# ChuWeiEr/GravInv3DHMC

Measured on AMD Instinct MI355X. Metric: HMC leapfrog steps/sec + G·ρ achieved HBM GB/s at 1/2/4/8 GPUs, higher is better.
Workload: dtype f64

## Files before the change

### gravinv3dhmc_amd/csrc/fold.hip.h

```cpp
#pragma once

namespace ghk {

struct FoldArgs {
    const double *S;
    const int *obs_img;
    const int *cell_orbit;
    int nF, ldF;
    int64_t n_orb;
    int64_t orb_per_team;
    int n_pp;
    int64_t N;
};

typedef const d2 __attribute__((address_space(1))) *gconst_d2ptr;

__global__ void __launch_bounds__(256) fold_build_kernel(const double *G, int64_t ld, FoldArgs f, double *S,
                                                         unsigned long long *dev_bits)
{
    __shared__ double red[2][4];
    const int64_t o = blockIdx.x;
    const int n = 4 * f.ldF;
    int co[4];
#pragma unroll
    for (int g = 0; g < 4; ++g) co[g] = f.cell_orbit[4 * o + g];
    double dev = 0.0, amax = 0.0;
    for (int e = threadIdx.x; e < n; e += blockDim.x) {
        const int i = e >> 2, k = e & 3;
        double mean = 0.0;
        if (i < f.nF) {
            double v[4];
#pragma unroll
            for (int g = 0; g < 4; ++g) v[g] = G[(int64_t)co[k ^ g] * ld + f.obs_img[4 * i + g]];
            mean = (((v[0] + v[1]) + v[2]) + v[3]) * 0.25;
#pragma unroll
            for (int g = 0; g < 4; ++g) dev = fmax(dev, fabs(v[g] - mean));
            amax = fmax(amax, fabs(mean));
        }
        S[o * n + e] = mean;
    }
#pragma unroll
    for (int off = 32; off >= 1; off >>= 1) {
        dev = fmax(dev, __shfl_xor(dev, off, WAVE));
        amax = fmax(amax, __shfl_xor(amax, off, WAVE));
    }
    const int lane = threadIdx.x & 63, wave = threadIdx.x >> 6;
    if (lane == 0) {
        red[0][wave] = dev;
        red[1][wave] = amax;
    }
    __syncthreads();
    if (threadIdx.x == 0) {
        for (int w = 1; w < (int)(blockDim.x >> 6); ++w) {
            dev = fmax(dev, red[0][w]);
            amax = fmax(amax, red[1][w]);
        }
        const double rel = amax > 0.0 ? dev / amax : 0.0;
        atomicMax(dev_bits, (unsigned long long)__double_as_longlong(rel));
    }
}

__device__ __forceinline__ double readlane_d(double v, int l)
{
    const long long b = __double_as_longlong(v);
    const int lo = __builtin_amdgcn_readlane((int)b, l);
    const int hi = __builtin_amdgcn_readlane((int)(b >> 32), l);
    return __longlong_as_double(((long long)hi << 32) | (long long)(unsigned)lo);
}

template <int EPT2>
struct FoldCol {
    d2 v[EPT2];
    int j;
    int jn;
    double cv;
};

constexpr int FOLD_SLOT = 16 * 16 + 8;

enum { FOLD_IN_X = 0, FOLD_IN_P, FOLD_IN_GREG, FOLD_IN_HI, FOLD_IN_LO, FOLD_IN_PN, FOLD_IN_GACC, FOLD_IN_N };

template <int CTRL>
__device__ __forceinline__ double dpp_mov(double v)
{
    const long long b = __double_as_longlong(v);
    const int lo = __builtin_amdgcn_update_dpp(0, (int)b, CTRL, 0xf, 0xf, false);
    const int hi = __builtin_amdgcn_update_dpp(0, (int)(b >> 32), CTRL, 0xf, 0xf, false);
    return __longlong_as_double(((long long)hi << 32) | (long long)(unsigned)lo);
}

template <int Q>
__device__ __forceinline__ double dpp_from_up(double v)
{
    const long long b = __double_as_longlong(v);
    const int lo = __builtin_amdgcn_update_dpp(0, (int)b, 0x100 | Q, 0xf, 0xf, false);
    const int hi = __builtin_amdgcn_update_dpp(0, (int)(b >> 32), 0x100 | Q, 0xf, 0xf, false);
    return __longlong_as_double(((long long)hi << 32) | (long long)(unsigned)lo);
}

template <int EPT2>
__global__ void __launch_bounds__(1024) fold_sweep_kernel(SweepArgs a, FoldArgs f)
{
    constexpr int TT = 1024, NW = 16;
    extern __shared__ __attribute__((aligned(16))) double smem[];
    double *rF = smem;
    double *scratch = smem + 4 * f.ldF;

    const int tid = threadIdx.x;
    const int lane = tid & 63;
    const int wave = tid >> 6;
    const int n2 = 2 * f.ldF;
    const int mode = a.mode;

    if (mode & SW_ADJ) {
        for (int e = tid; e < 4 * f.ldF; e += TT) rF[e] = (e >> 2) < f.nF ? a.r[f.obs_img[e]] : 0.0;
    }
    __syncthreads();

    const int64_t ob = (int64_t)blockIdx.x * f.orb_per_team;
    int64_t oend = ob + f.orb_per_team;
    if (oend > f.n_orb) oend = f.n_orb;
    const int cnt = ob < oend ? (int)(oend - ob) : 0;

    d2 acc[EPT2][2];
#pragma unroll
    for (int k = 0; k < EPT2; ++k) acc[k][0] = acc[k][1] = d2{0.0, 0.0};
    double pp = 0.0;

    unsigned voff = (unsigned)tid * (unsigned)sizeof(d2);
    unsigned coff_last;
    {
        const int e = (EPT2 - 1) * TT + tid;
        coff_last = (unsigned)(e < n2 ? e : n2 - 1) * (unsigned)sizeof(d2);
    }
    const bool last_in = (EPT2 - 1) * TT + tid < n2;
    const int hl = (lane >> 3) & 3, ql = lane & 7;
    const double *in_base = ql == FOLD_IN_P      ? a.p_in
                            : ql == FOLD_IN_GREG ? a.greg
                            : ql == FOLD_IN_HI   ? a.high
                            : ql == FOLD_IN_LO   ? a.low
                            : ql == FOLD_IN_PN   ? a.pn_in
                            : (ql == FOLD_IN_GACC && (mode & SW_GACC)) ? a.g_out
                                                                       : a.x_in;
    const int lastc = cnt - 1;
    auto orb = [&](int i) -> int64_t { return ob + (i < lastc ? i : lastc); };
    auto load_col = [&](FoldCol<EPT2> &c, int64_t o, int64_t o_after) {
        const int jn = f.cell_orbit[4 * o_after + hl];
        const unsigned long long col = (unsigned long long)(f.S + o * (int64_t)(4 * f.ldF));
#pragma unroll
        for (int k = 0; k < EPT2 - 1; ++k) {
            unsigned long long colk = col + (unsigned long long)k * TT * sizeof(d2);
            asm volatile("" : "+s"(colk));
            asm volatile("" : "+v"(voff));
            c.v[k] = __builtin_nontemporal_load(reinterpret_cast<gconst_d2ptr>(colk + voff));
        }
        asm volatile("" : "+v"(coff_last));
        c.v[EPT2 - 1] = __builtin_nontemporal_load(reinterpret_cast<gconst_d2ptr>(col + coff_last));
        asm volatile("" : "+v"(c.jn)::"memory");
        c.j = c.jn;
        c.cv = in_base[c.j];
        c.jn = jn;
    };

    auto process = [&](const FoldCol<EPT2> &cur, int it) {
        double xl = cur.cv;
        const double pl = dpp_from_up<FOLD_IN_P>(cur.cv);
        double xh[4];
        if (mode & SW_ADJ) {
            const d2 *rF2 = reinterpret_cast<const d2 *>(rF) + 2 * (tid >> 1);
            double u0 = 0.0, u1 = 0.0, u2 = 0.0, u3 = 0.0;
#pragma unroll
            for (int k = 0; k < EPT2; ++k) {
                if (k < EPT2 - 1 || last_in) {
                    const d2 ra = rF2[k * TT], rb = rF2[k * TT + 1];
                    const d2 v = cur.v[k];
                    u0 += v.x * ra.x;
                    u0 += v.y * ra.y;
                    u1 += v.x * ra.y;
                    u1 += v.y * ra.x;
                    u2 += v.x * rb.x;
                    u2 += v.y * rb.y;
                    u3 += v.x * rb.y;
                    u3 += v.y * rb.x;
                }
            }
            const bool odd = (tid & 1) != 0, hi2 = (tid & 2) != 0;
            const double w0 = odd ? u2 : u0, w1 = odd ? u3 : u1, w2 = odd ? u0 : u2, w3 = odd ? u1 : u3;
            const double a0 = (odd ? w2 : w0) + dpp_mov<0xb1>(odd ? w0 : w2);
            const double a1 = (odd ? w3 : w1) + dpp_mov<0xb1>(odd ? w1 : w3);
            double sq = (hi2 ? a1 : a0) + dpp_mov<0x4e>(hi2 ? a0 : a1);
            sq = dpp_add<0x114, 0xf>(sq);
            sq = dpp_add<0x118, 0xf>(sq);
            double *slot = scratch + (it & 1) * FOLD_SLOT;
            if ((lane & 15) >= 12) slot[wave * 16 + (((lane & 1) << 1) | ((lane >> 1) & 1)) * 4 + (lane >> 4)] = sq;
            __syncthreads();
            const d2 *sl = reinterpret_cast<const d2 *>(slot + (lane >> 2) * 16 + (lane & 3) * 4);
            const d2 ra = sl[0], rb = sl[1];
            double sv = (ra.x + ra.y) + (rb.x + rb.y);
            sv = dpp_add<0x114, 0xf>(sv);
            sv = dpp_add<0x118, 0xf>(sv);
            double t[4];
#pragma unroll
            for (int h = 0; h < 4; ++h)
                t[h] = ((readlane_d(sv, 12 + h) + readlane_d(sv, 28 + h)) + readlane_d(sv, 44 + h)) + readlane_d(sv, 60 + h);
            const double th = hl == 0 ? t[0] : hl == 1 ? t[1] : hl == 2 ? t[2] : t[3];
            const double g = 2.0 * th + dpp_from_up<FOLD_IN_GREG>(cur.cv);
            double pv = 0.0, pf = 0.0;
            if (mode & SW_PFIN) {
                pf = pl - a.c_p * g;
                pv = pf;
            }
            if (mode & SW_UPD) {
                const double chi = dpp_from_up<FOLD_IN_HI>(cur.cv), clo = dpp_from_up<FOLD_IN_LO>(cur.cv);
                const double psrc = (mode & SW_SPEC) ? dpp_from_up<FOLD_IN_PN>(cur.cv) : pl;
                double pj = psrc - a.c_u * g;
                double xj = xl + a.dt * pj;
                if (xj > chi) {
                    xj = chi;
                    pj = -pj;
                } else if (xj < clo) {
                    xj = clo;
                    pj = -pj;
                }
                pv = pj;
                xl = xj;
            }
            if (mode & SW_PFIN) {
#pragma unroll
                for (int h = 0; h < 4; ++h) {
                    const double q = readlane_d(pf, 8 * h);
                    pp += q * q;
                }
            }
            if (tid < 32 && ql == 0) {
                const int j = cur.j;
                if (mode & SW_GOUT) a.g_out[j] = (mode & SW_GACC) ? dpp_from_up<FOLD_IN_GACC>(cur.cv) + g : g;
                if (mode & SW_UPD) {
                    a.p_out[j] = pv;
                    a.x_out[j] = xl;
                } else if ((mode & SW_PFIN) && !(mode & SW_SPEC)) {
                    a.p_out[j] = pv;
                }
            }
        }
        if (mode & SW_FWD) {
#pragma unroll
            for (int h = 0; h < 4; ++h) xh[h] = readlane_d(xl, 8 * h);
#pragma unroll
            for (int k = 0; k < EPT2; ++k) {
                const d2 v = cur.v[k];
                acc[k][0].x += v.x * xh[0];
                acc[k][0].x += v.y * xh[1];
                acc[k][0].y += v.x * xh[1];
                acc[k][0].y += v.y * xh[0];
                acc[k][1].x += v.x * xh[2];
                acc[k][1].x += v.y * xh[3];
                acc[k][1].y += v.x * xh[3];
                acc[k][1].y += v.y * xh[2];
            }
        }
#pragma unroll
        for (int k = 0; k < EPT2; ++k) asm volatile("" ::"v"(cur.v[k]));
    };

    if (cnt > 0) {
        FoldCol<EPT2> b0, b1;
        b0.jn = f.cell_orbit[4 * orb(0) + hl];
        b1.jn = f.cell_orbit[4 * orb(1) + hl];
        load_col(b0, orb(0), orb(2));
        int i = 0;
        for (;;) {
            load_col(b1, orb(i + 1), orb(i + 3));
            process(b0, i);
            if (++i >= cnt) break;
            load_col(b0, orb(i + 1), orb(i + 3));
            process(b1, i);
            if (++i >= cnt) break;
        }
    }

    if ((mode & SW_PFIN) && tid == 0) {
        a.pp_part[blockIdx.x] = pp;
        for (int t = (int)(blockIdx.x + gridDim.x); t < f.n_pp; t += (int)gridDim.x) a.pp_part[t] = 0.0;
    }

    if (mode & SW_FWD) {
        double *out = a.slab + (int64_t)blockIdx.x * a.ld;
        double ds = 0.0;
#pragma unroll
        for (int k = 0; k < EPT2; ++k) {
            const int e = k * TT + tid;
            const double p2 = __shfl_xor(acc[k][1].x, 1, WAVE), p3 = __shfl_xor(acc[k][1].y, 1, WAVE);
            const double tA = acc[k][0].x + p2, tB = acc[k][0].y + p3;
            const int i = e >> 1;
            if (e < n2 && i < f.nF) {
                const int m2 = 2 * (tid & 1);
                out[f.obs_img[4 * i + m2]] = tA;
                out[f.obs_img[4 * i + m2 + 1]] = tB;
                ds += tA;
                ds += tB;
            }
        }
        for (int64_t e = f.N + tid; e < a.ld; e += TT) out[e] = 0.0;
        if (a.dsum) {
            const double t = block_allreduce_sum(ds, scratch, NW);
            if (tid == 0) a.dsum[blockIdx.x] = t;
        }
    }
}


struct FoldPairArgs {
    const int *wtab;
    const int *ptab;
    int64_t n_work, work_per_team;
};
constexpr int FOLD_PAIR_W = 16;
constexpr int FOLD_PSLOT = 64;

constexpr int fold_pair_slots(int rows) { return (rows - 1) / 2; }
constexpr int fold_pair_cols(int rows) { return 2 * (rows - fold_pair_slots(rows)); }

__global__ void __launch_bounds__(512) fold_pair_rows_kernel(FoldArgs f, const int *code, double *S)
{
    extern __shared__ __attribute__((aligned(16))) double smem[];
    const int n = 4 * f.ldF;
    double *blk = S + (int64_t)blockIdx.x * n;
    for (int e = threadIdx.x; e < n; e += blockDim.x) smem[e] = blk[e];
    __syncthreads();
    for (int e = threadIdx.x; e < n; e += blockDim.x) {
        const int cd = code[e >> 2];
        const int k = e >> 11, t = (e >> 2) & 511, w = min(512, f.ldF - 512 * k);
        blk[2048 * k + 2 * (((e >> 1) & 1) * w + t) + (e & 1)] = cd >= 0 ? smem[(cd & ~3) | ((e ^ cd) & 3)] : 0.0;
    }
}

__global__ void __launch_bounds__(256) fold_pair_mean_kernel(FoldArgs f, const int *row_tau, const int *orb_tau, double *S,
                                                             unsigned long long *dev_bits)
{
    __shared__ double red[2][4];
    const int64_t o = blockIdx.x;
    const int ot = orb_tau[o];
    const int64_t o2 = ot >> 2;
    const int co = ot & 3;
    const int n = 4 * f.nF;
    const int64_t ldb = 4 * (int64_t)f.ldF;
    double dev = 0.0, amax = 0.0;
    if (o <= o2) {
        for (int e = threadIdx.x; e < n; e += blockDim.x) {
            const int k = e & 3, rt = row_tau[e >> 2];
            const int ks = ((k & 1) << 1) | (k >> 1);
            const int e2 = (rt & ~3) | (ks ^ co ^ (rt & 3));
            if (o < o2 || e < e2) {
                const double u = S[o * ldb + e], v = S[o2 * ldb + e2];
                const double m = (u + v) * 0.5;
                S[o * ldb + e] = m;
                S[o2 * ldb + e2] = m;
                dev = fmax(dev, fabs(u - m));
                amax = fmax(amax, fabs(m));
            } else if (e == e2) {
                amax = fmax(amax, fabs(S[o * ldb + e]));
            }
        }
    }
#pragma unroll
    for (int off = 32; off >= 1; off >>= 1) {
        dev = fmax(dev, __shfl_xor(dev, off, WAVE));
        amax = fmax(amax, __shfl_xor(amax, off, WAVE));
    }
    const int lane = threadIdx.x & 63, wave = threadIdx.x >> 6;
    if (lane == 0) {
        red[0][wave] = dev;
        red[1][wave] = amax;
    }
    __syncthreads();
    if (threadIdx.x == 0) {
        for (int w = 1; w < (int)(blockDim.x >> 6); ++w) {
            dev = fmax(dev, red[0][w]);
            amax = fmax(amax, red[1][w]);
        }
        const double rel = amax > 0.0 ? dev / amax : 0.0;
        atomicMax(dev_bits, (unsigned long long)__double_as_longlong(rel));
    }
}

template <int ROWS>
struct FoldPairCol {
    d2 v[ROWS][2];
    int j;
    int jn, on;
    bool live;
    double cv;
};

template <int ROWS>
__global__ void __launch_bounds__(512) fold_pair_sweep_kernel(SweepArgs a, FoldArgs f, FoldPairArgs p)
{
    constexpr int TT = 512, NW = 8;
    constexpr int NP = fold_pair_slots(ROWS), NS = ROWS - NP, NC = fold_pair_cols(ROWS);
    extern __shared__ __attribute__((aligned(16))) double smem[];
    double *rL = smem;
    double *scratch = smem + NC * TT * 4;

    const int tid = threadIdx.x;
    const int lane = tid & 63;
    const int wave = tid >> 6;
    const int mode = a.mode;

    if (mode & SW_ADJ) {
        for (int e = tid; e < NC * TT * 4; e += TT) {
            const int i = p.ptab[e];
            rL[e] = i >= 0 ? a.r[i] : 0.0;
        }
    }
    __syncthreads();

    const int64_t wb = (int64_t)blockIdx.x * p.work_per_team;
    int64_t wend = wb + p.work_per_team;
    if (wend > p.n_work) wend = p.n_work;
    const int cnt = wb < wend ? (int)(wend - wb) : 0;

    d2 acc[NS][2][2];
#pragma unroll
    for (int s = 0; s < NS; ++s) acc[s][0][0] = acc[s][0][1] = acc[s][1][0] = acc[s][1][1] = d2{0.0, 0.0};
    double pp = 0.0;

    const int row_last = (ROWS - 1) * TT + tid;
    const bool last_in = row_last < f.ldF;
    const int w_last = f.ldF - (ROWS - 1) * TT;
    unsigned voff = (unsigned)tid * 16u;
    unsigned coff_last = (unsigned)(last_in ? tid : w_last - 1) * 16u;

    const int hl = (lane >> 3) & 3, ql = lane & 7, sl = lane >> 5;
    const double *in_base = ql == FOLD_IN_P      ? a.p_in
                            : ql == FOLD_IN_GREG ? a.greg
                            : ql == FOLD_IN_HI   ? a.high
                            : ql == FOLD_IN_LO   ? a.low
                            : ql == FOLD_IN_PN   ? a.pn_in
                            : (ql == FOLD_IN_GACC && (mode & SW_GACC)) ? a.g_out
                                                                       : a.x_in;
    const int lastc = cnt - 1;
    auto item = [&](int i) -> int64_t { return wb + (i < lastc ? i : lastc); };
    auto load_col = [&](FoldPairCol<ROWS> &c, int64_t w_after) {
        asm volatile("" : "+v"(c.jn), "+v"(c.on)::"memory");
        const int64_t o = __builtin_amdgcn_readfirstlane(c.on);
        c.live = c.jn >= 0;
        c.j = c.live ? c.jn : ~c.jn;
        asm volatile("" : "+v"(c.j));
        c.jn = p.wtab[FOLD_PAIR_W * w_after + (lane >> 3)];
        c.on = p.wtab[FOLD_PAIR_W * w_after + 8];
        const unsigned long long col = (unsigned long long)(f.S + o * (int64_t)(4 * f.ldF));
#pragma unroll
        for (int k = 0; k < ROWS - 1; ++k) {
            unsigned long long colk = col + (unsigned long long)k * TT * 32u, colh = colk + TT * 16u;
            asm volatile("" : "+s"(colk));
            asm volatile("" : "+s"(colh));
            asm volatile("" : "+v"(voff));
            c.v[k][0] = __builtin_nontemporal_load(reinterpret_cast<gconst_d2ptr>(colk + voff));
            c.v[k][1] = __builtin_nontemporal_load(reinterpret_cast<gconst_d2ptr>(colh + voff));
        }
        unsigned long long coll = col + (unsigned long long)(ROWS - 1) * TT * 32u, collh = coll + (unsigned)w_last * 16u;
        asm volatile("" : "+s"(coll));
        asm volatile("" : "+s"(collh));
        asm volatile("" : "+v"(coff_last));
        c.v[ROWS - 1][0] = __builtin_nontemporal_load(reinterpret_cast<gconst_d2ptr>(coll + coff_last));
        c.v[ROWS - 1][1] = __builtin_nontemporal_load(reinterpret_cast<gconst_d2ptr>(collh + coff_last));
        c.cv = in_base[c.j];
    };

    auto row_fma = [](const d2 v0, const d2 v1, const d2 wa, const d2 wb2, d2 &t01, d2 &t23) {
        t01.x += v0.x * wa.x;
        t01.x += v0.y * wa.y;
        t01.x += v1.x * wb2.x;
        t01.x += v1.y * wb2.y;
        t01.y += v0.x * wa.y;
        t01.y += v0.y * wa.x;
        t01.y += v1.x * wb2.y;
        t01.y += v1.y * wb2.x;
        t23.x += v0.x * wb2.x;
        t23.x += v0.y * wb2.y;
        t23.x += v1.x * wa.x;
        t23.x += v1.y * wa.y;
        t23.y += v0.x * wb2.y;
        t23.y += v0.y * wb2.x;
        t23.y += v1.x * wa.y;
        t23.y += v1.y * wa.x;
    };

    auto process = [&](const FoldPairCol<ROWS> &cur, int it) {
        double xl = cur.cv;
        const double pl = dpp_from_up<FOLD_IN_P>(cur.cv);
        if (mode & SW_ADJ) {
            const d2 *r2 = reinterpret_cast<const d2 *>(rL) + 2 * tid;
            d2 ua = d2{0.0, 0.0}, ub = ua, wa = ua, wb = ua;
#pragma unroll
            for (int s = 0; s < NS; ++s) {
                const int k = s < NP ? 2 * s : NP + s;
                if (k < ROWS - 1 || last_in) {
                    const d2 ra0 = r2[4 * s * TT], ra1 = r2[4 * s * TT + 1];
                    const d2 rb0 = r2[(4 * s + 2) * TT], rb1 = r2[(4 * s + 2) * TT + 1];
                    const d2 a0 = cur.v[k][0], a1 = cur.v[k][1];
                    row_fma(a0, a1, ra0, ra1, ua, ub);
                    row_fma(d2{a0.x, a1.x}, d2{a0.y, a1.y}, rb0, rb1, wa, wb);
                    if (s < NP) {
                        const d2 b0 = cur.v[k + 1][0], b1 = cur.v[k + 1][1];
                        row_fma(b0, b1, rb0, rb1, ua, ub);
                        row_fma(d2{b0.x, b1.x}, d2{b0.y, b1.y}, ra0, ra1, wa, wb);
                    }
                }
            }
            const bool odd = (lane & 1) != 0, hi2 = (lane & 2) != 0;
            const double u[4] = {ua.x, ua.y, ub.x, ub.y}, ut[4] = {wa.x, wb.x, wa.y, wb.y};
            double b[4];
#pragma unroll
            for (int q = 0; q < 4; ++q) b[q] = (odd ? ut[q] : u[q]) + dpp_mov<0xb1>(odd ? u[q] : ut[q]);
            double s0 = (hi2 ? b[2] : b[0]) + dpp_mov<0x4e>(hi2 ? b[0] : b[2]);
            double s1 = (hi2 ? b[3] : b[1]) + dpp_mov<0x4e>(hi2 ? b[1] : b[3]);
            s0 = dpp_add<0x114, 0xf>(s0);
            s0 = dpp_add<0x118, 0xf>(s0);
            s1 = dpp_add<0x114, 0xf>(s1);
            s1 = dpp_add<0x118, 0xf>(s1);
            s0 += __shfl_xor(s0, 16, WAVE);
            s1 += __shfl_xor(s1, 16, WAVE);
            s0 += __shfl_xor(s0, 32, WAVE);
            s1 += __shfl_xor(s1, 32, WAVE);
            double *slot = scratch + (it & 1) * FOLD_PSLOT;
            if (lane >= 12 && lane < 16) {
                const int c = lane - 12;
                *reinterpret_cast<d2 *>(slot + wave * 8 + 4 * (c & 1) + 2 * (c >> 1)) = d2{s0, s1};
            }
            __syncthreads();
            double sv = slot[lane];
            sv = dpp_add<0x118, 0xf>(sv);
            sv += __shfl_xor(sv, 16, WAVE);
            sv += __shfl_xor(sv, 32, WAVE);
            const double th = __shfl(sv, 8 + 4 * sl + hl, WAVE);
            const double g = 2.0 * th + dpp_from_up<FOLD_IN_GREG>(cur.cv);
            double pv = 0.0, pf = 0.0;
            if (mode & SW_PFIN) {
                pf = pl - a.c_p * g;
                pv = pf;
            }
            if (mode & SW_UPD) {
                const double chi = dpp_from_up<FOLD_IN_HI>(cur.cv), clo = dpp_from_up<FOLD_IN_LO>(cur.cv);
                const double psrc = (mode & SW_SPEC) ? dpp_from_up<FOLD_IN_PN>(cur.cv) : pl;
                double pj = psrc - a.c_u * g;
                double xj = xl + a.dt * pj;
                if (xj > chi) {
                    xj = chi;
                    pj = -pj;
                } else if (xj < clo) {
                    xj = clo;
                    pj = -pj;
                }
                pv = pj;
                xl = xj;
            }
            if (mode & SW_PFIN) {
                const double pz = cur.live ? pf : 0.0;
#pragma unroll
                for (int h = 0; h < 8; ++h) {
                    const double q = readlane_d(pz, 8 * h);
                    pp += q * q;
                }
            }
            if (tid < 64 && ql == 0 && cur.live) {
                const int j = cur.j;
                if (mode & SW_GOUT) a.g_out[j] = (mode & SW_GACC) ? dpp_from_up<FOLD_IN_GACC>(cur.cv) + g : g;
                if (mode & SW_UPD) {
                    a.p_out[j] = pv;
                    a.x_out[j] = xl;
                } else if ((mode & SW_PFIN) && !(mode & SW_SPEC)) {
                    a.p_out[j] = pv;
                }
            }
        }
        if (mode & SW_FWD) {
            const double xz = cur.live ? xl : 0.0;
            const d2 xa = d2{readlane_d(xz, 0), readlane_d(xz, 8)}, xb = d2{readlane_d(xz, 16), readlane_d(xz, 24)};
            const d2 ya = d2{readlane_d(xz, 32), readlane_d(xz, 40)}, yb = d2{readlane_d(xz, 48), readlane_d(xz, 56)};
            const d2 ysa = d2{ya.x, yb.x}, ysb = d2{ya.y, yb.y};
#pragma unroll
            for (int s = 0; s < NS; ++s) {
                const int k = s < NP ? 2 * s : NP + s;
                const d2 a0 = cur.v[k][0], a1 = cur.v[k][1];
                row_fma(a0, a1, xa, xb, acc[s][0][0], acc[s][0][1]);
                row_fma(d2{a0.x, a1.x}, d2{a0.y, a1.y}, ysa, ysb, acc[s][1][0], acc[s][1][1]);
                if (s < NP) {
                    const d2 b0 = cur.v[k + 1][0], b1 = cur.v[k + 1][1];
                    row_fma(b0, b1, xa, xb, acc[s][1][0], acc[s][1][1]);
                    row_fma(d2{b0.x, b1.x}, d2{b0.y, b1.y}, ysa, ysb, acc[s][0][0], acc[s][0][1]);
                }
            }
        }
#pragma unroll
        for (int k = 0; k < ROWS; ++k) {
            asm volatile("" ::"v"(cur.v[k][0]));
            asm volatile("" ::"v"(cur.v[k][1]));
        }
    };

    if (cnt > 0) {
        FoldPairCol<ROWS> b0, b1, b2;
        b0.jn = p.wtab[FOLD_PAIR_W * item(0) + (lane >> 3)];
        b0.on = p.wtab[FOLD_PAIR_W * item(0) + 8];
        b1.jn = p.wtab[FOLD_PAIR_W * item(1) + (lane >> 3)];
        b1.on = p.wtab[FOLD_PAIR_W * item(1) + 8];
        b2.jn = p.wtab[FOLD_PAIR_W * item(2) + (lane >> 3)];
        b2.on = p.wtab[FOLD_PAIR_W * item(2) + 8];
        load_col(b0, item(3));
        load_col(b1, item(4));
        int i = 0;
        for (; i + 2 < cnt; i += 3) {
            load_col(b2, item(i + 5));
            process(b0, i);
            load_col(b0, item(i + 6));
            process(b1, i + 1);
            load_col(b1, item(i + 7));
            process(b2, i + 2);
        }
        if (i < cnt) process(b0, i);
        if (i + 1 < cnt) process(b1, i + 1);
    }

    if ((mode & SW_PFIN) && tid == 0) {
        a.pp_part[blockIdx.x] = pp;
        for (int t = (int)(blockIdx.x + gridDim.x); t < f.n_pp; t += (int)gridDim.x) a.pp_part[t] = 0.0;
    }

    if (mode & SW_FWD) {
        double *out = a.slab + (int64_t)blockIdx.x * a.ld;
        const int4 *pt = reinterpret_cast<const int4 *>(p.ptab) + tid;
        double ds = 0.0;
#pragma unroll
        for (int c = 0; c < NC; ++c) {
            if ((c & 1) && (c >> 1) >= NP) continue;
            const int4 oi = pt[c * TT];
            if (oi.x >= 0) {
                const d2 s01 = acc[c >> 1][c & 1][0], s23 = acc[c >> 1][c & 1][1];
                out[oi.x] = s01.x;
                out[oi.y] = s01.y;
                out[oi.z] = s23.x;
                out[oi.w] = s23.y;
                ds += s01.x;
                ds += s01.y;
                ds += s23.x;
                ds += s23.y;
            }
        }
        for (int64_t e = f.N + tid; e < a.ld; e += TT) out[e] = 0.0;
        __syncthreads();
#pragma unroll
        for (int s = NP; s < NS; ++s) {
            const int4 oi = pt[(2 * s + 1) * TT];
            if (oi.x >= 0) {
                const d2 s01 = acc[s][1][0], s23 = acc[s][1][1];
                out[oi.x] += s01.x;
                out[oi.y] += s01.y;
                out[oi.z] += s23.x;
                out[oi.w] += s23.y;
                ds += s01.x;
                ds += s01.y;
                ds += s23.x;
                ds += s23.y;
            }
        }
        if (a.dsum) {
            const double t = block_allreduce_sum(ds, scratch, NW);
            if (tid == 0) a.dsum[blockIdx.x] = t;
        }
    }
}

}
```

### gravinv3dhmc_amd/csrc/host_fold.h

```cpp
#pragma once


namespace fold_detail {

struct Axis {
    std::vector<double> lo, hi;
    double tol = 0.0;
    void build(std::vector<double> v, double t)
    {
        tol = t;
        std::sort(v.begin(), v.end());
        for (double x : v) {
            if (lo.empty() || x - hi.back() > tol) {
                lo.push_back(x);
                hi.push_back(x);
            } else {
                hi.back() = x;
            }
        }
    }
    int find(double x) const
    {
        const size_t k = (size_t)(std::upper_bound(lo.begin(), lo.end(), x + tol) - lo.begin());
        if (k == 0) return -1;
// ... 123 lines not shown
        idx.v.reserve((size_t)M);
        for (int64_t j = 0; j < M; ++j) {
            const double *b = b6 + 6 * j;
            keys[(size_t)j] = Key{ax.find(b[0]), ax.find(b[1]), ay.find(b[2]), ay.find(b[3]), bits(b[4]), bits(b[5])};
            idx.v.push_back({keys[(size_t)j], (int)j});
        }
        if (!idx.build()) return GH_FOLD_CELLS;
        for (int64_t j = 0; j < M; ++j) {
            const Key &k = keys[(size_t)j];
            if (mx[(size_t)k[0]] < 0 || mx[(size_t)k[1]] < 0 || my[(size_t)k[2]] < 0 || my[(size_t)k[3]] < 0)
                return GH_FOLD_CELLS;
            csx[(size_t)j] = idx.find(Key{mx[(size_t)k[1]], mx[(size_t)k[0]], k[2], k[3], k[4], k[5]});
            csy[(size_t)j] = idx.find(Key{k[0], k[1], my[(size_t)k[3]], my[(size_t)k[2]], k[4], k[5]});
            if (csx[(size_t)j] < 0 || csy[(size_t)j] < 0) return GH_FOLD_CELLS;
        }
    }
    int rc = orbits(osx, osy, obs_img);
    if (rc != GH_FOLD_ON) return rc == GH_FOLD_CELLS ? GH_FOLD_OBS : rc;
    return orbits(csx, csy, cell_orbit);
}

static int fold_pair_detect_host(int64_t N, const double *x, const double *y, const double *z, int64_t M, const double *b6,
                                 const std::vector<int> &obs_img, const std::vector<int> &cell_orbit, std::vector<int> &obs_tau,
                                 std::vector<int> &cell_tau, std::vector<int> &row_tau, std::vector<int> &orb_tau,
                                 std::vector<int> &work)
{
    using namespace fold_detail;
    double xmin = b6[0], xmax = b6[1], ymin = b6[2], ymax = b6[3];
    for (int64_t j = 0; j < M; ++j) {
        const double *b = b6 + 6 * j;
        xmin = std::min(xmin, std::min(b[0], b[1]));
        xmax = std::max(xmax, std::max(b[0], b[1]));
        ymin = std::min(ymin, std::min(b[2], b[3]));
        ymax = std::max(ymax, std::max(b[2], b[3]));
    }
    double mag = std::max(std::max(std::fabs(xmin), std::fabs(xmax)), std::max(std::fabs(ymin), std::fabs(ymax)));
    for (int64_t i = 0; i < N; ++i) mag = std::max(mag, std::max(std::fabs(x[i]), std::fabs(y[i])));
    const double tol = 8.0 * DBL_EPSILON * mag;
    const double cx = 0.5 * (xmin + xmax), cy = 0.5 * (ymin + ymax);
    auto across = [](const Axis &from, double cf, const Axis &to, double ct, std::vector<int> &m) {
        m.assign(from.lo.size(), -1);
        for (size_t q = 0; q < from.lo.size(); ++q) m[q] = to.find(ct + (0.5 * (from.lo[q] + from.hi[q]) - cf));
    };

    obs_tau.assign((size_t)N, -1);
    {
        Axis ax, ay;
        ax.build(std::vector<double>(x, x + N), tol);
        ay.build(std::vector<double>(y, y + N), tol);
        std::vector<int> x2y, y2x;
        across(ax, cx, ay, cy, x2y);
        across(ay, cy, ax, cx, y2x);
        std::vector<int> qx((size_t)N), qy((size_t)N);
        Index idx;
        idx.v.reserve((size_t)N);
        for (int64_t i = 0; i < N; ++i) {
            qx[(size_t)i] = ax.find(x[i]);
            qy[(size_t)i] = ay.find(y[i]);
            idx.v.push_back({Key{qx[(size_t)i], qy[(size_t)i], bits(z[i]), 0, 0, 0}, (int)i});
        }
        if (!idx.build()) return GH_FOLD_PAIR_OBS;
        for (int64_t i = 0; i < N; ++i) {
            const int a = y2x[(size_t)qy[(size_t)i]], b = x2y[(size_t)qx[(size_t)i]];
            if (a < 0 || b < 0) return GH_FOLD_PAIR_OBS;
            if ((obs_tau[(size_t)i] = idx.find(Key{a, b, bits(z[i]), 0, 0, 0})) < 0) return GH_FOLD_PAIR_OBS;
        }
    }
    cell_tau.assign((size_t)M, -1);
    {
        Axis ax, ay;
        std::vector<double> vx, vy;
        vx.reserve(2 * (size_t)M);
        vy.reserve(2 * (size_t)M);
        for (int64_t j = 0; j < M; ++j) {
            vx.push_back(b6[6 * j]);
            vx.push_back(b6[6 * j + 1]);
            vy.push_back(b6[6 * j + 2]);
            vy.push_back(b6[6 * j + 3]);
        }
        ax.build(std::move(vx), tol);
        ay.build(std::move(vy), tol);
        std::vector<int> x2y, y2x;
        across(ax, cx, ay, cy, x2y);
        across(ay, cy, ax, cx, y2x);
        std::vector<Key> keys((size_t)M);
        Index idx;
        idx.v.reserve((size_t)M);
        for (int64_t j = 0; j < M; ++j) {
            const double *b = b6 + 6 * j;
            keys[(size_t)j] = Key{ax.find(b[0]), ax.find(b[1]), ay.find(b[2]), ay.find(b[3]), bits(b[4]), bits(b[5])};
            idx.v.push_back({keys[(size_t)j], (int)j});
        }
        if (!idx.build()) return GH_FOLD_PAIR_CELLS;
        for (int64_t j = 0; j < M; ++j) {
            const Key &k = keys[(size_t)j];
            const int a0 = y2x[(size_t)k[2]], a1 = y2x[(size_t)k[3]], b0 = x2y[(size_t)k[0]], b1 = x2y[(size_t)k[1]];
            if (a0 < 0 || a1 < 0 || b0 < 0 || b1 < 0) return GH_FOLD_PAIR_CELLS;
            if ((cell_tau[(size_t)j] = idx.find(Key{a0, a1, b0, b1, k[4], k[5]})) < 0) return GH_FOLD_PAIR_CELLS;
        }
    }
    auto rows = [](const std::vector<int> &img, const std::vector<int> &tau, std::vector<int> &rt) {
        const size_t n = img.size();
        std::vector<int> pos(n);
        for (size_t e = 0; e < n; ++e) pos[(size_t)img[e]] = (int)e;
        rt.assign(n / 4, -1);
        for (size_t e = 0; e < n; ++e) {
            const int i = img[e], g = (int)(e & 3);
            if (tau[(size_t)tau[(size_t)i]] != i) return false;
            const int at = pos[(size_t)tau[(size_t)i]] ^ (((g & 1) << 1) | (g >> 1));
            if (g == 0) rt[e >> 2] = at;
            if (rt[e >> 2] != at) return false;
        }
        return true;
    };
    if (!rows(obs_img, obs_tau, row_tau)) return GH_FOLD_PAIR_OBS;
    if (!rows(cell_orbit, cell_tau, orb_tau)) return GH_FOLD_PAIR_CELLS;
    work.clear();
    for (size_t o = 0; o < orb_tau.size(); ++o) {
        const int o2 = orb_tau[o] >> 2;
        if (o2 == (int)o) {
            work.push_back((int)o);
            work.push_back(-1);
        } else if ((int)o < o2) {
            work.push_back((int)o);
            work.push_back(o2);
        }
    }
    return GH_FOLD_PAIR_ON;
}

namespace fold_detail {

struct PairRows {
    int rows = 0, pair_slots = 0, cols = 0;
    int64_t pairs_in_slots = 0, pairs_split = 0, self_rows = 0;
    std::vector<int> code, ptab;
};

inline bool pair_rows_plan(int nF, int ldF, const std::vector<int> &obs_img, const std::vector<int> &row_tau, PairRows &pr)
{
    constexpr int TT = 512;
    pr.rows = (ldF + TT - 1) / TT;
    pr.pair_slots = ghk::fold_pair_slots(pr.rows);
    pr.cols = ghk::fold_pair_cols(pr.rows);
    pr.pairs_in_slots = pr.pairs_split = pr.self_rows = 0;
    pr.code.assign((size_t)ldF, -1);
    pr.ptab.assign((size_t)pr.cols * TT * 4, -1);
    auto place = [&](int s, int t, int k, int f, bool both) {
        const int rt = row_tau[(size_t)f], f2 = rt >> 2, cf = rt & 3;
        int *pa = pr.ptab.data() + ((size_t)(2 * s) * TT + (size_t)t) * 4, *pb = pa + (size_t)TT * 4;
        for (int g = 0; g < 4; ++g) {
            pa[g] = obs_img[4 * (size_t)f + g];
            pb[g] = obs_img[4 * (size_t)f2 + (g ^ cf)];
        }
        pr.code[(size_t)k * TT + t] = 4 * f;
        if (both) pr.code[(size_t)(k + 1) * TT + t] = 4 * f2 + cf;
    };
    const int64_t cap = (int64_t)pr.pair_slots * TT;
    int64_t lone = 0;
    auto place_lone = [&](int f) -> bool {
        const int64_t n = 2 * cap + lone;
        if (n >= ldF) return false;
        const int l = (int)(lone / TT), t = (int)(lone % TT);
        place(pr.pair_slots + l, t, 2 * pr.pair_slots + l, f, false);
        ++lone;
        return true;
    };
    int64_t np = 0;
    for (int f = 0; f < nF; ++f) {
        const int f2 = row_tau[(size_t)f] >> 2;
        if (f2 <= f) continue;
        if (np < cap) {
            place((int)(np / TT), (int)(np % TT), 2 * (int)(np / TT), f, true);
            ++pr.pairs_in_slots;
        } else {
            if (!place_lone(f) || !place_lone(f2)) return false;
            ++pr.pairs_split;
        }
        ++np;
    }
    for (int f = 0; f < nF; ++f) {
        if ((row_tau[(size_t)f] >> 2) != f) continue;
        if (!place_lone(f)) return false;
        ++pr.self_rows;
    }
    return true;
}

}

constexpr int FOLD_PAIR_MAX_ROWS = 5;

static int fold_pair_tables(gh_ctx *c, const double *ox, const double *oy, const double *oz, const double *b6)
{
    gh_ctx::Fold &f = c->fd;
    std::vector<int> obs_tau, cell_tau, row_tau, orb_tau, work;
    f.pair_on = false;
    f.n_work = f.n_pairs = 0;
    f.pair_reason = fold_pair_detect_host(c->N, ox, oy, oz, c->M, b6, f.obs_img, f.cell_orbit, obs_tau, cell_tau, row_tau,
                                          orb_tau, work);
    f.pair_detected = f.pair_reason == GH_FOLD_PAIR_ON;
    if (!f.pair_detected) return GH_OK;
    f.pair_reason = GH_FOLD_PAIR_UNDECIDED;
    f.n_work = (int64_t)(work.size() / 2);
    std::vector<int> wtab((size_t)f.n_work * ghk::FOLD_PAIR_W, 0);
    for (int64_t w = 0; w < f.n_work; ++w) {
        const int o = work[2 * (size_t)w], o2 = work[2 * (size_t)w + 1];
        int *t = wtab.data() + w * ghk::FOLD_PAIR_W;
        for (int h = 0; h < 4; ++h) {
            t[h] = f.cell_orbit[4 * (size_t)o + h];
            t[4 + h] = o2 >= 0 ? cell_tau[(size_t)t[h]] : ~t[h];
        }
        t[8] = o;
        f.n_pairs += o2 >= 0;
    }
    fold_detail::PairRows pr;
    f.pair_rows_ok = f.ldF <= 512 * FOLD_PAIR_MAX_ROWS && fold_detail::pair_rows_plan(f.nF, f.ldF, f.obs_img, row_tau, pr);
    if (!f.pair_rows_ok) {
        pr.code.assign((size_t)f.ldF, -1);
        pr.ptab.assign(4, -1);
    }
    auto up = [&](int **d, const std::vector<int> &h, size_t cap) -> int {
        TRY(dalloc(c, d, cap, false));
        HIPCHK(c, hipMemcpyAsync(*d, h.data(), sizeof(int) * h.size(), hipMemcpyHostToDevice, c->stream));
        return GH_OK;
    };
    TRY(up(&f.wtab_d, wtab, (size_t)f.n_orb * ghk::FOLD_PAIR_W));
    TRY(up(&f.ptab_d, pr.ptab, (size_t)ghk::fold_pair_cols(FOLD_PAIR_MAX_ROWS) * 512 * 4));
    TRY(up(&f.row_code_d, pr.code, (size_t)f.ldF));
    TRY(up(&f.row_tau_d, row_tau, (size_t)f.nF));
    TRY(up(&f.orb_tau_d, orb_tau, (size_t)f.n_orb));
    HIPCHK(c, hipStreamSynchronize(c->stream));
    return GH_OK;
}

static int fold_detect(gh_ctx *c)
{
    gh_ctx::Fold &f = c->fd;
    f.detected = -1;
    f.valid = false;
    f.gen = ~0ull;
    f.reason = GH_FOLD_NOT_GZ;
    f.pair_detected = f.pair_on = false;
    f.pair_reason = GH_FOLD_PAIR_NO_FOLD;
    if (c->cell_kind != GH_CELL_PRISM || c->joint || c->mf || !c->G) return GH_OK;
    std::vector<double> ox((size_t)c->N), oy((size_t)c->N), oz((size_t)c->N), b6((size_t)c->M * 6);
    TRY(d2h(c, ox.data(), c->obs[0], ox.size()));
    TRY(d2h(c, oy.data(), c->obs[1], oy.size()));
    TRY(d2h(c, oz.data(), c->obs[2], oz.size()));
    TRY(d2h(c, b6.data(), c->bounds, b6.size()));
    f.reason = fold_detect_host(c->N, ox.data(), oy.data(), oz.data(), c->M, b6.data(), f.obs_img, f.cell_orbit);
    if (f.reason != GH_FOLD_ON) return GH_OK;
    f.nF = (int)(c->N / 4);
    f.ldF = (f.nF + 15) / 16 * 16;
    f.n_orb = c->M / 4;
    TRY(dalloc(c, &f.obs_img_d, (size_t)c->N, false));
    TRY(dalloc(c, &f.cell_orbit_d, (size_t)c->M, false));
    HIPCHK(c, hipMemcpyAsync(f.obs_img_d, f.obs_img.data(), sizeof(int) * f.obs_img.size(), hipMemcpyHostToDevice, c->stream));
    HIPCHK(c, hipMemcpyAsync(f.cell_orbit_d, f.cell_orbit.data(), sizeof(int) * f.cell_orbit.size(), hipMemcpyHostToDevice,
                             c->stream));
    HIPCHK(c, hipStreamSynchronize(c->stream));
    TRY(fold_pair_tables(c, ox.data(), oy.data(), oz.data(), b6.data()));
    f.detected = 1;
    f.reason = GH_FOLD_UNDECIDED;
    return GH_OK;
}


constexpr int FOLD_MAX_EPT2 = 5;
constexpr double FOLD_MAX_DEV = 1e-7;

typedef void (*fold_fn)(SweepArgs, FoldArgs);

static fold_fn fold_kernel_for(int ept2)
{
    switch (ept2) {
    case 1: return fold_sweep_kernel<1>;
    case 2: return fold_sweep_kernel<2>;
    case 3: return fold_sweep_kernel<3>;
    case 4: return fold_sweep_kernel<4>;
    case 5: return fold_sweep_kernel<5>;
    }
    return nullptr;
}

typedef void (*fold_pair_fn)(SweepArgs, FoldArgs, FoldPairArgs);

static fold_pair_fn fold_pair_kernel_for(int rows)
{
    switch (rows) {
    case 1: return fold_pair_sweep_kernel<1>;
    case 2: return fold_pair_sweep_kernel<2>;
    case 3: return fold_pair_sweep_kernel<3>;
    case 4: return fold_pair_sweep_kernel<4>;
    case 5: return fold_pair_sweep_kernel<5>;
    }
    return nullptr;
}

constexpr size_t FOLD_PAIR_MAX_LDS = 160u << 10;

static size_t fold_pair_lds_limit(const gh_ctx *c)
{
    return ((size_t)8 * c->fd.nF + 2 * FOLD_PSLOT) * sizeof(double);
}

static size_t fold_pair_lds(const gh_ctx *c)
{
    return ((size_t)ghk::fold_pair_cols(c->fd.pair_rows) * 512 * 4 + 2 * FOLD_PSLOT) * sizeof(double);
}

static int64_t fold_store_bytes(const gh_ctx *c)
{
    return c->fd.n_orb * 4 * (int64_t)c->fd.ldF * (int64_t)sizeof(double);
}

static FoldArgs fold_args(const gh_ctx *c)
{
    const gh_ctx::Fold &f = c->fd;
    FoldArgs a{};
    a.S = f.S;
    a.obs_img = f.obs_img_d;
    a.cell_orbit = f.cell_orbit_d;
    a.nF = f.nF;
    a.ldF = f.ldF;
    a.n_orb = f.n_orb;
    a.orb_per_team = f.orb_per_team;
    a.n_pp = c->n_teams;
    a.N = c->N;
    return a;
}

static FoldPairArgs fold_pair_args(const gh_ctx *c)
{
    const gh_ctx::Fold &f = c->fd;
    FoldPairArgs p{};
    p.wtab = f.wtab_d;
    p.ptab = f.ptab_d;
    p.n_work = f.n_work;
    p.work_per_team = f.work_per_team;
    return p;
}

static int64_t fold_sweep_bytes(const gh_ctx *c)
{
    const gh_ctx::Fold &f = c->fd;
    return (f.pair_on ? f.n_work : f.n_orb) * 4 * (int64_t)f.ldF * (int64_t)sizeof(double);
}

static int fold_build(gh_ctx *c)
{
    gh_ctx::Fold &f = c->fd;
    const auto t0 = std::chrono::steady_clock::now();
    TRY(dalloc(c, &f.S, (size_t)(fold_store_bytes(c) / (int64_t)sizeof(double)), false));
    TRY(dalloc(c, &f.dev_bits, 1, false));
    TRY(dalloc(c, &f.zeros, (size_t)c->M));
    HIPCHK(c, hipMemsetAsync(f.dev_bits, 0, sizeof(unsigned long long), c->stream));
    fold_build_kernel<<<dim3((unsigned)f.n_orb), dim3(256), 0, c->stream>>>(c->G, c->ld, fold_args(c), f.S, f.dev_bits);
    HIPCHK(c, hipGetLastError());
    unsigned long long bits = 0;
    HIPCHK(c, hipMemcpyAsync(&bits, f.dev_bits, sizeof bits, hipMemcpyDeviceToHost, c->stream));
    HIPCHK(c, hipStreamSynchronize(c->stream));
    memcpy(&f.max_dev, &bits, sizeof bits);
    if (f.pair_on) {
        HIPCHK(c, hipMemsetAsync(f.dev_bits, 0, sizeof(unsigned long long), c->stream));
        fold_pair_mean_kernel<<<dim3((unsigned)f.n_orb), dim3(256), 0, c->stream>>>(fold_args(c), f.row_tau_d, f.orb_tau_d, f.S,
                                                                                   f.dev_bits);
        HIPCHK(c, hipGetLastError());
        HIPCHK(c, hipMemcpyAsync(&bits, f.dev_bits, sizeof bits, hipMemcpyDeviceToHost, c->stream));
        HIPCHK(c, hipStreamSynchronize(c->stream));
        double d8 = 0.0;
        memcpy(&d8, &bits, sizeof bits);
        f.max_dev += d8;
        const size_t blk = (size_t)4 * f.ldF * sizeof(double);
        HIPCHK(c, allow_dynamic_lds(reinterpret_cast<const void *>(fold_pair_rows_kernel), blk));
        fold_pair_rows_kernel<<<dim3((unsigned)f.n_orb), dim3(512), blk, c->stream>>>(fold_args(c), f.row_code_d, f.S);
        HIPCHK(c, hipGetLastError());
        HIPCHK(c, hipStreamSynchronize(c->stream));
    }
    f.build_ms = std::chrono::duration<double, std::milli>(std::chrono::steady_clock::now() - t0).count();
    return GH_OK;
}

static int fold_use(gh_ctx *c, bool *use)
{
    gh_ctx::Fold &f = c->fd;
    *use = false;
    if (f.detected != 1 || f.exact) return GH_OK;
    if (c->sh.kind != 0 || c->wv.on || c->joint || c->mf || c->n_panels != 1) {
        f.reason = GH_FOLD_PATH;
        return GH_OK;
    }
    if (f.gen == c->G_gen) {
        *use = f.valid;
        return GH_OK;
    }
    f.gen = c->G_gen;
    f.valid = false;
    f.pair_on = false;
    if (env_int("GRAVHMC_FOLD", 1) == 0) {
        f.reason = GH_FOLD_SWITCHED_OFF;
        return GH_OK;
    }
    const int64_t min_mb = env_int("GRAVHMC_FOLD_MIN_MB", 512);
    if (c->ld * c->M * (int64_t)sizeof(double) <= (min_mb << 20)) {
        f.reason = GH_FOLD_SMALL;
        return GH_OK;
    }
    f.ept2 = (2 * f.ldF + 1023) / 1024;
    if (f.ept2 > FOLD_MAX_EPT2 || (c->ld <= 1024 && env_int("GRAVHMC_RESIDENT", 1) != 0)) {
        f.reason = GH_FOLD_PATH;
        return GH_OK;
    }
    {
        size_t free_b = 0, total_b = 0;
        (void)hipMemGetInfo(&free_b, &total_b);
        if (!f.S && (int64_t)free_b < fold_store_bytes(c) + ((int64_t)256 << 20)) {
            f.reason = GH_FOLD_NOMEM;
            return GH_OK;
        }
    }
    f.pair_on = false;
    f.pair_rows = (f.ldF + 511) / 512;
    if (!f.pair_detected) {
    } else if (env_int("GRAVHMC_FOLD_PAIR", 1) == 0) {
        f.pair_reason = GH_FOLD_PAIR_SWITCHED_OFF;
    } else if (fold_pair_lds_limit(c) > FOLD_PAIR_MAX_LDS || f.pair_rows > FOLD_PAIR_MAX_ROWS || !f.pair_rows_ok) {
        f.pair_reason = GH_FOLD_PAIR_ROWS;
    } else if (allow_dynamic_lds(reinterpret_cast<const void *>(fold_pair_kernel_for(f.pair_rows)), fold_pair_lds(c)) !=
               hipSuccess) {
        (void)hipGetLastError();
        f.pair_reason = GH_FOLD_PAIR_ROWS;
    } else {
        f.pair_on = true;
        f.pair_reason = GH_FOLD_PAIR_ON;
    }
    const void *fn = f.pair_on ? reinterpret_cast<const void *>(fold_pair_kernel_for(f.pair_rows))
                               : reinterpret_cast<const void *>(fold_kernel_for(f.ept2));
    const int threads = f.pair_on ? 512 : 1024;
    f.lds = f.pair_on ? fold_pair_lds(c) : ((size_t)4 * f.ldF + 2 * FOLD_SLOT) * sizeof(double);
    HIPCHK(c, allow_dynamic_lds(fn, f.lds));
    int occ = 0;
    if (hipOccupancyMaxActiveBlocksPerMultiprocessor(&occ, fn, threads, f.lds) != hipSuccess || occ < 1) {
        (void)hipGetLastError();
        occ = 1;
    }
    const int64_t items = f.pair_on ? f.n_work : f.n_orb;
    int grid = (int)std::min<int64_t>(std::min<int64_t>((int64_t)c->cus * occ, c->grid), items);
    const int64_t per_team = (items + grid - 1) / grid;
    f.orb_per_team = f.work_per_team = per_team;
    f.grid = (int)((items + per_team - 1) / per_team);
    TRY(fold_build(c));
    if (!(f.max_dev <= FOLD_MAX_DEV)) {
        f.reason = GH_FOLD_DEVIATION;
        return GH_OK;
    }
    f.valid = true;
    f.reason = GH_FOLD_ON;
    *use = true;
    return GH_OK;
}

struct FoldExact {
    gh_ctx *c;
    explicit FoldExact(gh_ctx *c_) : c(c_) { c->fd.exact = true; }
    ~FoldExact() { c->fd.exact = false; }
};

static int launch_fold(gh_ctx *c, SweepArgs &a)
{
    gh_ctx::Fold &f = c->fd;
    a.ld = c->ld;
    a.M = c->M;
    a.row0 = 0;
    a.rows = c->ld;
    bool timed = c->prof && c->ev_used + 2 <= c->ev.size() && (c->prof_seen++ % c->prof_stride) == 0;
    if (timed) HIPCHK(c, hipEventRecord(c->ev[c->ev_used], c->stream));
    SweepArgs b = a;
    for (const double **v : {&b.x_in, &b.p_in, &b.low, &b.high, &b.greg, &b.pn_in})
        if (!*v) *v = f.zeros;
    if (f.pair_on)
        hipLaunchKernelGGL(fold_pair_kernel_for(f.pair_rows), dim3(f.grid), dim3(512), f.lds, c->stream, b, fold_args(c),
                           fold_pair_args(c));
    else
        hipLaunchKernelGGL(fold_kernel_for(f.ept2), dim3(f.grid), dim3(1024), f.lds, c->stream, b, fold_args(c));
    if (timed) {
        HIPCHK(c, hipEventRecord(c->ev[c->ev_used + 1], c->stream));
        c->ev_bytes[c->ev_used / 2] = fold_sweep_bytes(c);
        c->ev_used += 2;
    }
    if (c->prof) c->prof_launches += 1;
    f.launches += 1;
    HIPCHK(c, hipGetLastError());
    return GH_OK;
}
```

### profiles/summarize.py

```python
#!/usr/bin/env python3
import csv
import glob
import json
import os
import subprocess
import sys


def find(d, pat):
    return sorted(glob.glob(os.path.join(d, "**", pat), recursive=True))


def stats(d, out):
    rows = []
    for f in find(d, "*kernel_stats.csv"):
        rows += list(csv.DictReader(open(f)))
    rows.sort(key=lambda r: -float(r["TotalDurationNs"]))
    keys = ["Name", "Calls", "TotalDurationNs", "AverageNs", "Percentage", "MinNs", "MaxNs", "StdDev"]
    with open(out, "w", newline="") as fh:
        w = csv.DictWriter(fh, fieldnames=keys, quoting=csv.QUOTE_NONNUMERIC)
        w.writeheader()
        for r in rows:
            w.writerow({k: r[k] for k in keys})


def pmc(out, note, dirs):
    acc = {}
    for d in dirs:
        for f in find(d, "*counter_collection.csv"):
            for r in csv.DictReader(open(f)):
                k = acc.setdefault(r["Kernel_Name"], {}).setdefault(r["Counter_Name"], [])
                k.append(float(r["Counter_Value"]))
    kernels = {}
    for name, counters in sorted(acc.items()):
        e = {}
        for c, vals in sorted(counters.items()):
            e[c + "_avg"] = sum(vals) / len(vals)
            e["dispatches_" + c] = len(vals)
        if "FETCH_SIZE_avg" in e:
            e["hbm_read_bytes"] = 2.0 * 1024.0 * e["FETCH_SIZE_avg"]
        if "WRITE_SIZE_avg" in e:
            e["hbm_write_bytes"] = 1024.0 * e["WRITE_SIZE_avg"]
        if "SQ_BUSY_CYCLES_avg" in e and "SQ_ACTIVE_INST_VALU_avg" in e and e.get("SQ_WAVE_CYCLES_avg"):
            e["valu_active_share_of_wave_cycles"] = e["SQ_ACTIVE_INST_VALU_avg"] / e["SQ_WAVE_CYCLES_avg"]
        kernels[name] = e
    commit = os.environ.get("GRAVHMC_PROFILED_COMMIT")
    if not commit:
        try:
            commit = subprocess.check_output(["git", "rev-parse", "--short", "HEAD"], text=True,
                                             cwd=os.path.dirname(os.path.abspath(__file__))).strip()
        except Exception:
            commit = "n/a"
    json.dump({"note": note, "commit": commit, "kernels": kernels}, open(out, "w"), indent=1)


if __name__ == "__main__":
    if sys.argv[1] == "stats":
        stats(sys.argv[2], sys.argv[3])
    else:
        pmc(sys.argv[2], sys.argv[3], sys.argv[4:])
```

Before: 985.1.

## Overlap adjoint residual gather with column prefetch and simplify cross-wave reduction

Moves the adjoint residual staging into LDS after the first work-table and column prefetch loads are issued. It now uses vectorised int4 index loads and register staging, so the gather latency overlaps with the initial column loads instead of stalling before them. The per-iteration cross-wave reduction drops the xor-16/32 shuffles and writes partial sums to a larger swizzled LDS slot (FOLD_PSLOT 64→256). Each lane then reads pairs and finishes with DPP row adds. This raises LDS scratch use and adds register pressure from the staged residuals. A timing-series profiling helper is also added.

```diff
diff --git a/gravinv3dhmc_amd/csrc/fold.hip.h b/gravinv3dhmc_amd/csrc/fold.hip.h
--- a/gravinv3dhmc_amd/csrc/fold.hip.h
+++ b/gravinv3dhmc_amd/csrc/fold.hip.h
@@ -316,7 +316,7 @@
     int64_t n_work, work_per_team;
 };
 constexpr int FOLD_PAIR_W = 16;
-constexpr int FOLD_PSLOT = 64;
+constexpr int FOLD_PSLOT = 256;
 
 constexpr int fold_pair_slots(int rows) { return (rows - 1) / 2; }
 constexpr int fold_pair_cols(int rows) { return 2 * (rows - fold_pair_slots(rows)); }
@@ -407,14 +407,6 @@
     const int wave = tid >> 6;
     const int mode = a.mode;
 
-    if (mode & SW_ADJ) {
-        for (int e = tid; e < NC * TT * 4; e += TT) {
-            const int i = p.ptab[e];
-            rL[e] = i >= 0 ? a.r[i] : 0.0;
-        }
-    }
-    __syncthreads();
-
     const int64_t wb = (int64_t)blockIdx.x * p.work_per_team;
     int64_t wend = wb + p.work_per_team;
     if (wend > p.n_work) wend = p.n_work;
@@ -431,7 +423,10 @@
     unsigned voff = (unsigned)tid * 16u;
     unsigned coff_last = (unsigned)(last_in ? tid : w_last - 1) * 16u;
 
-    const int hl = (lane >> 3) & 3, ql = lane & 7, sl = lane >> 5;
+    const int ql = lane & 7;
+    const int ex_d0 = 4 * (lane & 1) + (lane & 2);
+    const int ex_w = 128 * (lane >> 5) + 2 * (8 * ex_d0 + (wave ^ (ex_d0 >> 1))) + ((lane >> 4) & 1);
+    const int ex_r = 2 * (lane ^ (lane >> 4));
     const double *in_base = ql == FOLD_IN_P      ? a.p_in
                             : ql == FOLD_IN_GREG ? a.greg
                             : ql == FOLD_IN_HI   ? a.high
@@ -439,8 +434,9 @@
                             : ql == FOLD_IN_PN   ? a.pn_in
                             : (ql == FOLD_IN_GACC && (mode & SW_GACC)) ? a.g_out
                                                                        : a.x_in;
-    const int lastc = cnt - 1;
-    auto item = [&](int i) -> int64_t { return wb + (i < lastc ? i : lastc); };
+    const int lastc = cnt > 0 ? cnt - 1 : 0;
+    const int64_t wfirst = cnt > 0 ? wb : 0;
+    auto item = [&](int i) -> int64_t { return wfirst + (i < lastc ? i : lastc); };
     auto load_col = [&](FoldPairCol<ROWS> &c, int64_t w_after) {
         asm volatile("" : "+v"(c.jn), "+v"(c.on)::"memory");
         const int64_t o = __builtin_amdgcn_readfirstlane(c.on);
@@ -520,22 +516,18 @@
             s0 = dpp_add<0x118, 0xf>(s0);
             s1 = dpp_add<0x114, 0xf>(s1);
             s1 = dpp_add<0x118, 0xf>(s1);
-            s0 += __shfl_xor(s0, 16, WAVE);
-            s1 += __shfl_xor(s1, 16, WAVE);
-            s0 += __shfl_xor(s0, 32, WAVE);
-            s1 += __shfl_xor(s1, 32, WAVE);
             double *slot = scratch + (it & 1) * FOLD_PSLOT;
-            if (lane >= 12 && lane < 16) {
-                const int c = lane - 12;
-                *reinterpret_cast<d2 *>(slot + wave * 8 + 4 * (c & 1) + 2 * (c >> 1)) = d2{s0, s1};
+            if ((lane & 12) == 12) {
+                slot[ex_w] = s0;
+                slot[ex_w + 16] = s1;
             }
             __syncthreads();
-            double sv = slot[lane];
-            sv = dpp_add<0x118, 0xf>(sv);
-            sv += __shfl_xor(sv, 16, WAVE);
-            sv += __shfl_xor(sv, 32, WAVE);
-            const double th = __shfl(sv, 8 + 4 * sl + hl, WAVE);
-            const double g = 2.0 * th + dpp_from_up<FOLD_IN_GREG>(cur.cv);
+            const d2 p01 = *reinterpret_cast<const d2 *>(slot + ex_r), p23 = *reinterpret_cast<const d2 *>(slot + 128 + ex_r);
+            double sv = (p01.x + p01.y) + (p23.x + p23.y);
+            sv = dpp_add<0x101, 0xf>(sv);
+            sv = dpp_add<0x102, 0xf>(sv);
+            sv = dpp_add<0x104, 0xf>(sv);
+            const double g = 2.0 * sv + dpp_from_up<FOLD_IN_GREG>(cur.cv);
             double pv = 0.0, pf = 0.0;
             if (mode & SW_PFIN) {
                 pf = pl - a.c_p * g;
@@ -600,16 +592,42 @@
         }
     };
 
+    const bool adj = (mode & SW_ADJ) != 0;
+    const int4 *pt0 = reinterpret_cast<const int4 *>(p.ptab) + tid;
+    int4 ro[NC];
+    d2 rv[NC][2];
+    if (adj) {
+#pragma unroll
+        for (int c = 0; c < NC; ++c) ro[c] = pt0[c * TT];
+    }
+    FoldPairCol<ROWS> b0, b1, b2;
+    b0.jn = p.wtab[FOLD_PAIR_W * item(0) + (lane >> 3)];
+    b0.on = p.wtab[FOLD_PAIR_W * item(0) + 8];
+    b1.jn = p.wtab[FOLD_PAIR_W * item(1) + (lane >> 3)];
+    b1.on = p.wtab[FOLD_PAIR_W * item(1) + 8];
+    b2.jn = p.wtab[FOLD_PAIR_W * item(2) + (lane >> 3)];
+    b2.on = p.wtab[FOLD_PAIR_W * item(2) + 8];
+    asm volatile("" : "+v"(b0.jn), "+v"(b0.on), "+v"(b1.jn), "+v"(b1.on), "+v"(b2.jn), "+v"(b2.on)::"memory");
+    if (adj) {
+#pragma unroll
+        for (int c = 0; c < NC; ++c) {
+            rv[c][0] = d2{a.r[max(ro[c].x, 0)], a.r[max(ro[c].y, 0)]};
+            rv[c][1] = d2{a.r[max(ro[c].z, 0)], a.r[max(ro[c].w, 0)]};
+        }
+    }
+    load_col(b0, item(3));
+    load_col(b1, item(4));
+    if (adj) {
+        d2 *r2 = reinterpret_cast<d2 *>(rL) + 2 * tid;
+#pragma unroll
+        for (int c = 0; c < NC; ++c) {
+            r2[2 * c * TT] = d2{ro[c].x >= 0 ? rv[c][0].x : 0.0, ro[c].y >= 0 ? rv[c][0].y : 0.0};
+            r2[2 * c * TT + 1] = d2{ro[c].z >= 0 ? rv[c][1].x : 0.0, ro[c].w >= 0 ? rv[c][1].y : 0.0};
+        }
+    }
+    __syncthreads();
+
     if (cnt > 0) {
-        FoldPairCol<ROWS> b0, b1, b2;
-        b0.jn = p.wtab[FOLD_PAIR_W * item(0) + (lane >> 3)];
-        b0.on = p.wtab[FOLD_PAIR_W * item(0) + 8];
-        b1.jn = p.wtab[FOLD_PAIR_W * item(1) + (lane >> 3)];
-        b1.on = p.wtab[FOLD_PAIR_W * item(1) + 8];
-        b2.jn = p.wtab[FOLD_PAIR_W * item(2) + (lane >> 3)];
-        b2.on = p.wtab[FOLD_PAIR_W * item(2) + 8];
-        load_col(b0, item(3));
-        load_col(b1, item(4));
         int i = 0;
         for (; i + 2 < cnt; i += 3) {
             load_col(b2, item(i + 5));
diff --git a/gravinv3dhmc_amd/csrc/host_fold.h b/gravinv3dhmc_amd/csrc/host_fold.h
--- a/gravinv3dhmc_amd/csrc/host_fold.h
+++ b/gravinv3dhmc_amd/csrc/host_fold.h
@@ -449,7 +449,7 @@
 
 static size_t fold_pair_lds_limit(const gh_ctx *c)
 {
-    return ((size_t)8 * c->fd.nF + 2 * FOLD_PSLOT) * sizeof(double);
+    return ((size_t)8 * c->fd.nF + 2 * 64) * sizeof(double);
 }
 
 static size_t fold_pair_lds(const gh_ctx *c)
diff --git a/profiles/summarize.py b/profiles/summarize.py
--- a/profiles/summarize.py
+++ b/profiles/summarize.py
@@ -54,8 +54,36 @@
     json.dump({"note": note, "commit": commit, "kernels": kernels}, open(out, "w"), indent=1)
 
 
+def series(out, pattern, note, labelled):
+    skip = 40
+    res = {"note": note, "skip": skip}
+    for item in labelled:
+        label, d = item.split("=", 1)
+        rows = []
+        for f in find(d, "*kernel_trace.csv"):
+            rows += [r for r in csv.DictReader(open(f)) if pattern in r["Kernel_Name"]]
+        rows.sort(key=lambda r: int(r["Start_Timestamp"]))
+        ns = [int(r["End_Timestamp"]) - int(r["Start_Timestamp"]) for r in rows]
+        tail = ns[skip:]
+        med = sorted(tail)[len(tail) // 2] if tail else 0
+        fused = [(i, v) for i, v in enumerate(tail) if v >= 0.93 * med]
+        short = [(skip + i, v) for i, v in enumerate(tail) if v < 0.93 * med]
+        vals = [v for _, v in fused]
+        n = len(vals)
+        mean = sum(vals) / n if n else 0.0
+        var = sum((v - mean) ** 2 for v in vals) / (n - 1) if n > 1 else 0.0
+        even = [v for i, v in fused if i % 2 == 0]
+        odd = [v for i, v in fused if i % 2 == 1]
+        res[label] = {"ns": ns, "fused_n": n, "fused_mean_ns": mean, "fused_stderr_ns": (var / n) ** 0.5 if n else 0.0,
+                      "fused_sigma_ns": var ** 0.5, "short_sweeps_index_ns": short,
+                      "odd_even_half_diff_ns": 0.5 * abs(sum(odd) / len(odd) - sum(even) / len(even)) if odd and even else 0.0}
+    json.dump(res, open(out, "w"), indent=1)
+
+
 if __name__ == "__main__":
     if sys.argv[1] == "stats":
         stats(sys.argv[2], sys.argv[3])
+    elif sys.argv[1] == "series":
+        series(sys.argv[2], sys.argv[3], sys.argv[4], sys.argv[5:])
     else:
         pmc(sys.argv[2], sys.argv[3], sys.argv[4:])
```

Result: faster. 1015, median of 6 (+3.0%).
